# d3sm0/gym_pomdp

Measured on AMD Instinct MI355X. Metric: env steps/sec (whole node), RockSample(7,8) batch=2^20, 1/2/4/8 MI355X, higher is better.
Workload: dtype int32

## Files before the change

### gym_pomdp_amd/csrc/envs/rock.hip.h

```cpp
#pragma once
#include "../envs_common.hip.h"

namespace pomdp {

template <int W, bool STOCH = false>
struct RockEnv {
    using Params = pomdp_rock_params;
    using Reward = int32_t;
    using S = typename std::conditional<W == 1, uint32_t, uint64_t>::type;
    static constexpr int WORDS = W;
    static constexpr const char *NAME = STOCH ? (W == 1 ? "StochasticRockEnv<1>" : "StochasticRockEnv<2>") : (W == 1 ? "RockEnv<1>" : "RockEnv<2>");
    static constexpr bool POOLED_LPT2 = !STOCH;
    static constexpr bool QUAD_STEP = true;
    static constexpr bool HAS_ROCKS = true;
    static constexpr bool POOLED_ANY_LPT = !STOCH;
    static constexpr bool STOCHASTIC = STOCH;
    static constexpr bool QUAD_TAB = true;
    struct Shared {
        uint2 thr[32];
        int8_t grid[256];
        uint8_t rxy[16];
        uint16_t rpos[16];
        uint32_t dir_y[16];
        uint32_t dir_x[16];
// ... 44 lines not shown
        sh.row[tid] = same;
    }

    static __device__ __forceinline__ void load(State &st, const uint32_t *state, int64_t n, uint32_t i)
    {
        st.s = ld_stream(state + i);
        if (W == 2) st.s |= (S)((uint64_t)ld_stream(state + n + i) << 32);
    }
    static __device__ __forceinline__ void store(const State &st, uint32_t *state, int64_t n, uint32_t i, bool)
    {
        st_stream(state + i, (uint32_t)st.s);
        if (W == 2) st_stream(state + n + i, (uint32_t)((uint64_t)st.s >> 32));
    }

    static __device__ __forceinline__ uint32_t elem(const uint4 &w, uint32_t e) { return e == 0 ? w.x : e == 1 ? w.y : e == 2 ? w.z : w.w; }

    template <class LowWord>
    static __device__ __forceinline__ bool k53_le(uint32_t H, uint32_t th, uint32_t tl, LowWord lo)
    {
        const uint32_t kh = H >> 5;
        bool r = kh < th;
        if (kh == th) r = (lo() >> 6) <= tl;
        return r;
    }
    static __device__ __forceinline__ uint32_t rock_code_hi(uint32_t H)
    {
        const uint32_t kh = H >> 5;
        return kh > HALF_HI ? 2u : (kh < HALF_HI ? 0u : 3u);
    }
    static __device__ __forceinline__ uint32_t rock_code_lo(uint32_t L) { return (L >> 6) ? 2u : 1u; }
    template <bool AUTO = false>
    static __device__ __forceinline__ uint4 reset_block(const RngKey &key, uint32_t lane, uint32_t j2)
    {
        const uint32_t c3 = AUTO ? (((uint32_t)POMDP_STREAM_STEP << 24) | (SENSOR_BLOCK + j2)) : (((uint32_t)POMDP_STREAM_RESET << 24) | j2);
        return philox4x32_10(lane >> 2, key.t_lo, key.t_hi, c3, key.k0, key.k1);
    }
    template <bool AUTO>
    static __device__ __forceinline__ uint32_t reset_codes(const RngKey &key, uint32_t lane, int K)
    {
        return reset_codes<AUTO>(elem(reset_block<AUTO>(key, lane, 0u), lane & 3u), key, lane, K);
    }
    template <bool AUTO>
    static __device__ __forceinline__ uint32_t reset_codes(uint32_t w, const RngKey &key, uint32_t lane, int K)
    {
        uint32_t codes = w & 0xAAAAAAAAu;
        if (__popc(w) <= 6) reset_ties<AUTO>(w, key, lane, K, codes, 0);
        return codes & (K >= 16 ? 0xFFFFFFFFu : ((1u << (2 * K)) - 1u));
    }
    template <bool AUTO>
    static __device__ __forceinline__ void reset_ties(uint32_t w, const RngKey &key, uint32_t lane, int K, uint32_t &word, int base)
    {
        bool have_lo = false;
        uint32_t l = 0;
        for (int j = 0; j < K; ++j) {
            const uint32_t rot = (uint32_t)(2 * j + 2) & 31u;
            if (rock_code_hi(__builtin_rotateright32(w, rot)) != 3u) continue;
            if (!have_lo) {
                uint32_t lane_ = lane;
                asm volatile("" : "+v"(lane_));
                l = elem(reset_block<AUTO>(rare_key(key), lane_, 1u), lane & 3u);
                have_lo = true;
            }
            const uint32_t c = rock_code_lo(__builtin_rotateright32(l, rot));
            word = (word & ~(3u << (base + 2 * j))) | (c << (base + 2 * j));
        }
    }
    static __device__ __forceinline__ uint4 quad_block(const RngKey &key, uint32_t lane, uint32_t j2)
    {
        return philox4x32_10(lane >> 2, key.t_lo, key.t_hi, ((uint32_t)POMDP_STREAM_STEP << 24) | j2, key.k0, key.k1);
    }

    static __device__ __forceinline__ void reset_codes4(const uint32_t (&R)[4], const RngKey &key, uint32_t first, int K,
                                                        uint32_t (&codes)[4])
    {
        const uint32_t exist = K >= 16 ? 0xFFFFFFFFu : ((1u << (2 * K)) - 1u);
#pragma unroll
        for (int e = 0; e < 4; ++e) codes[e] = R[e] & 0xAAAAAAAAu & exist;
        if (min(min(__popc(R[0]), __popc(R[1])), min(__popc(R[2]), __popc(R[3]))) <= 6) {
#pragma unroll
            for (int e = 0; e < 4; ++e) codes[e] = reset_codes<true>(R[e], key, first + (uint32_t)e, K);
        }
    }
    static constexpr int RESET_NUMERIC_K = 8;
    static __device__ __forceinline__ uint32_t reset_tie_bound(int K) { return 1u << (2 * min(K, RESET_NUMERIC_K) + 5); }
    template <int N, bool ROT, bool NUMERIC>
    static __device__ __forceinline__ void fresh_states(const uint32_t (&R)[N], const RngKey &key, uint32_t first, int K,
                                                        uint32_t start, uint32_t bound, uint32_t (&fresh)[N])
    {
        const uint32_t exist = K >= 16 ? 0xFFFFFFFFu : ((1u << (2 * K)) - 1u);
        auto word = [&](uint32_t codes) { return ROT ? (codes | start) : (start | (codes << 8)); };
#pragma unroll
        for (int e = 0; e < N; ++e) fresh[e] = word(R[e] & (0xAAAAAAAAu & exist));
        bool look;
        if constexpr (NUMERIC) {
            uint32_t least = R[0];
#pragma unroll
            for (int e = 1; e < N; ++e) least = min(least, R[e]);
            look = least < bound;
        } else {
            int fewest = __popc(R[0]);
#pragma unroll
            for (int e = 1; e < N; ++e) fewest = min(fewest, (int)__popc(R[e]));
            look = fewest <= 6;
        }
        if (look) {
#pragma unroll
            for (int e = 0; e < N; ++e)
                if (__popc(R[e]) <= 6) reset_ties<true>(R[e], key, first + (uint32_t)e, K, fresh[e], ROT ? 0 : 8);
        }
    }
    static __device__ __forceinline__ int reset(const Shared &, const Params &p, State &st, const RngKey &key,
                                                uint32_t lane)
    {
        const uint64_t s = (uint32_t)p.start_x | ((uint32_t)p.start_y << 4);
        st.s = (S)(s | ((uint64_t)reset_codes<false>(key, lane, p.num_rocks) << 8));
        return 0;
    }
    static __device__ __forceinline__ int reset_ob(const Params &, const State &) { return 0; }

    static __device__ __forceinline__ void reset_where(const Shared &, const Params &p, State &st, bool fresh,
                                                       const RngKey &key, uint32_t lane)
    {
        if (!__any(fresh)) return;
        const uint32_t codes = reset_codes<true>(key, lane, p.num_rocks);
        if (fresh) st.s = (S)((uint64_t)((uint32_t)p.start_x | ((uint32_t)p.start_y << 4)) | ((uint64_t)codes << 8));
    }
    static __device__ __forceinline__ void reset_where_chain(const Shared &sh, const Params &p, State &st, bool fresh,
                                                             const RngKey &key, uint32_t lane, const RngKey &akey,
                                                             uint32_t n_actions, int &next_action)
    {
        reset_where_chain_default<RockEnv>(sh, p, st, fresh, key, lane, akey, n_actions, next_action);
    }
    static __device__ __forceinline__ S fresh_state(const Params &p, uint32_t w, const RngKey &key, uint32_t lane)
    {
        return (S)((uint64_t)((uint32_t)p.start_x | ((uint32_t)p.start_y << 4)) | ((uint64_t)reset_codes<true>(w, key, lane, p.num_rocks) << 8));
    }

    static __device__ __forceinline__ int legal_count(const Shared &sh, const Params &p, const State &st, uint32_t &pre,
                                                      int &n_pre, uint32_t &alive)
    {
        const S s = st.s;
        const int x = (int)(s & 15u), y = (int)((s >> 4) & 15u), K = p.num_rocks;
        pre = 1u; n_pre = 1;
        if (y + 1 < p.size) { pre |= 0u << (3 * n_pre); ++n_pre; }
        if (y - 1 >= 0) { pre |= 2u << (3 * n_pre); ++n_pre; }
        if (x - 1 >= 0) { pre |= 3u << (3 * n_pre); ++n_pre; }
        const int id = sh.grid[x * 16 + y];
        if (id >= 0 && id < K && ((uint32_t)(s >> (8 + 2 * (id & 15))) & 3u) != 1u) { pre |= 4u << (3 * n_pre); ++n_pre; }
        const uint64_t r = (uint64_t)s >> 8;
        const uint64_t even = 0x5555555555555555ull;
        const uint64_t spread = ~(r & ~(r >> 1)) & even & ((1ull << (2 * K)) - 1ull);
        alive = (uint32_t)spread;
        return n_pre + __popc(alive);
    }
    struct Legal { uint32_t pre, alive; int n_pre, count; };
    static __device__ __forceinline__ Legal legal_set(const Shared &sh, const Params &p, const State &st)
    {
        Legal L;
        L.count = legal_count(sh, p, st, L.pre, L.n_pre, L.alive);
        return L;
    }
    static __device__ __forceinline__ int legal_pick(const Shared &sh, const Legal &L, int idx)
    {
        if (idx < L.n_pre) return (int)((L.pre >> (3 * idx)) & 7u);
        const int j = nth_set_bit<2>(L.alive, idx - L.n_pre) >> 1;
        const uint32_t rxy = sh.rxy[j & 15];
        return 5 + sh.grid[(rxy & 15u) * 16 + (rxy >> 4)];
    }
    static __device__ __forceinline__ int legal_nth(const Shared &sh, const Params &p, const State &st, int idx)
    {
        return legal_pick(sh, legal_set(sh, p, st), idx);
    }
    static __device__ __forceinline__ int legal_count(const Shared &sh, const Params &p, const State &st)
    {
        uint32_t pre, alive; int n_pre;
        return legal_count(sh, p, st, pre, n_pre, alive);
    }

    static __device__ __forceinline__ bool check_ok(int measured, int count, double pv)
    {
        return measured < 5 && abs(count) < 2 && 0 < pv && pv < 1;
    }
    static __device__ __forceinline__ void belief_update(const Shared &sh, const Params &p, const State &st, int a, int ob,
                                                         const pomdp_rock_belief &b, int64_t n, uint32_t i, uint32_t &ck)
    {
        const S s = st.s;
        const int x = (int)(s & 15u), y = (int)((s >> 4) & 15u), r = (a - 5) & 15;
        const uint32_t rxy = sh.rxy[r];
        const double eff = p.eff[abs(x - (int)(rxy & 15u)) + abs(y - (int)(rxy >> 4))];
        const int64_t k = (int64_t)r * n + i;
        double lkv = b.lkv[k], lkw = b.lkw[k];
// ... 47 lines not shown
        uint32_t m = (alive & ck) << 5;
        if (y + 1 < p.size && north) m |= 1u << 0;
        if (east) m |= 1u << 1;
        if (y - 1 >= 0 && south) m |= 1u << 2;
        if (x - 1 >= 0 && west) m |= 1u << 3;
        return m;
    }

    static __device__ __forceinline__ int select_target(const Shared &sh, const Params &p, const State &st,
                                                        const pomdp_rock_belief &b, int64_t n, uint32_t i)
    {
        const S s = st.s;
        const int x = (int)(s & 15u), y = (int)((s >> 4) & 15u), K = p.num_rocks;
        int best = 4 * p.size * p.size, best_rock = -1;
        for (int j = 0; j < K; ++j) {
            if (((uint32_t)(s >> (8 + 2 * j)) & 3u) == 1u || b.count[(int64_t)j * n + i] < 0) continue;
            const uint32_t rxy = sh.rxy[j];
            const int dx = x - (int)(rxy & 15u), dy = y - (int)(rxy >> 4), d2 = dx * dx + dy * dy;
            if (d2 < best) { best = d2; best_rock = j; }
        }
        return best_rock;
    }

    static __device__ __forceinline__ double compute_prob(const Shared &sh, const Params &p, const State &st, int a, int ob)
    {
        if (a <= 4) return ob == 0 ? 1.0 : 0.0;
        const S s = st.s;
        const int x = (int)(s & 15u), y = (int)((s >> 4) & 15u), r = (a - 5) & 15;
        const uint32_t rxy = sh.rxy[r];
        const double eff = p.eff[abs(x - (int)(rxy & 15u)) + abs(y - (int)(rxy >> 4))];
        const uint32_t code = (uint32_t)(s >> (8 + 2 * r)) & 3u;
        if ((ob == 2 && code == 2u) || (ob == 1 && code == 0u)) return eff;
        return 1 - eff;
    }

    template <class RT>
    static __device__ __forceinline__ void step_pre(const Shared &sh, const Params &p, State &st, int a, RT &rew,
                                                    int &done, Aux &aux)
    {
        const S s = st.s;
        const uint32_t x = (uint32_t)s & 15u, y = ((uint32_t)s >> 4) & 15u;
        const uint32_t size = (uint32_t)p.size, K = (uint32_t)p.num_rocks;
        const int r = (a - 5) & 15;
        const uint32_t rp = sh.rpos[r];
        const uint32_t d = __builtin_amdgcn_sad_u8(x | (y << 8), rp, 0u);
        aux.th = sh.thr[d].x;
        aux.r = (uint8_t)r;
        aux.good = ((uint32_t)(s >> (8 + 2 * r)) & 3u) == 2u;
        aux.want = a > 4;
        const int penalty = STOCH ? 0 : -100;
        const int id = sh.grid[x * 16 + y];
        const int sh_ = 8 + 2 * (id & 15);
        const uint32_t code = (uint32_t)(s >> sh_) & 3u;
        const bool sample_ok = ((uint32_t)id < K) & (code != 1u);
        const uint32_t a2 = (uint32_t)a << 1;
        const uint32_t nx = x + (uint32_t)__builtin_amdgcn_sbfe(0xC4, a2, 2u), ny = y + (uint32_t)__builtin_amdgcn_sbfe(0x31, a2, 2u);
        const bool inside = max(nx, ny) < size;
        const bool is_move = a < 4, is_sample = a == 4, east = a == 1;
        const bool moved = is_move & inside, left = is_move & !inside, sampled = is_sample & sample_ok,
                   missed = is_sample & !sample_ok;
        const uint32_t d_move = ((uint32_t)s & 0xFFu) ^ (nx | (ny << 4));
        const S d_sample = (S)(code ^ 1u) << sh_;
        st.s = s ^ (moved ? (S)d_move : (sampled ? d_sample : (S)0));
        const bool good_rock = code == 2u;
        int rw = ((left & east) | (sampled & good_rock)) ? 10 : 0;
        rw = (sampled & !good_rock) ? -10 : rw;
        rw = ((left & !east) | missed) ? penalty : rw;
        rew = rw;
        if (STOCH) done = left & east;
        else done = left | missed;
    }
    static __device__ __forceinline__ uint32_t thr_lo_of(const Shared &sh, const State &st, int r)
    {
        const uint32_t x = (uint32_t)st.s & 15u, y = ((uint32_t)st.s >> 4) & 15u;
        return sh.thr[__builtin_amdgcn_sad_u8(x | (y << 8), sh.rpos[r & 15], 0u)].y;
    }
    static constexpr int TAB_ACTIONS = W == 1 ? 17 : 21;

    static constexpr uint32_t REC_LUT_LO = 0x0A0A9CF6u, REC_LUT_HI = 0x00000000u;
    using TabEntry = typename std::conditional<W == 1, uint2, uint32_t>::type;
    struct RecTab { TabEntry e[TAB_ACTIONS][256]; };
    static constexpr uint32_t REC_ROCK = 1u << 31;
    static constexpr uint32_t TIE_SPAN = 32u;
    static __device__ __forceinline__ uint32_t rec_thr_word(uint32_t T) { return T >= (1u << 27) ? 0xFFFFFFFFu : T << 5; }
    static __device__ __forceinline__ uint32_t rec_f(uint32_t off, int c, uint32_t ob_mask, uint32_t oc)
    {
        const uint32_t rbyte = (((uint64_t)REC_LUT_HI << 32 | REC_LUT_LO) >> (8u * oc)) & 0xFFu;
        return off | (((uint32_t)c & 3u) << 5) | (ob_mask << 8) | (rbyte << 16) | ((oc & 1u) << 24);
    }
    static constexpr uint32_t ROT_POS = 24u;
    template <bool ROT = false>
    static __device__ __forceinline__ void build_rec_tab(RecTab &tab, const Shared &sh, const Params &p, int pos)
    {
        static_assert(!ROT || W == 1, "the rotated layout is the one-state-word loops'");
        constexpr uint32_t POS0 = ROT ? ROT_POS : 0u, ROCK0 = ROT ? 0u : 8u;
        const uint32_t x = (uint32_t)pos & 15u, y = (uint32_t)pos >> 4, size = (uint32_t)p.size, K = (uint32_t)p.num_rocks;
        const int id = sh.grid[x * 16 + y];
        const uint32_t NOTHING = 6u << 28, PENALTY = (STOCH ? 6u : 1u) << 28, EXIT_EAST = 3u << 28;
        const uint32_t NO_TIE = 1u << 27;
        for (int a = 0; a < 5 + (int)K && a < TAB_ACTIONS; ++a) {
            uint32_t e, f;
            if (a < 4) {
                const uint32_t nx = x + (uint32_t)((a == 1) - (a == 3)), ny = y + (uint32_t)((a == 0) - (a == 2));
                const bool inside = max(nx, ny) < size;
                e = inside ? (((uint32_t)pos ^ (nx | (ny << 4))) | NOTHING) : (a == 1 ? EXIT_EAST : PENALTY);
                e |= NO_TIE;
                f = rec_f(POS0 + ((a & 1) ? 0u : 4u), inside ? (a < 2 ? 1 : -1) : 0, 0u, e >> 28 & 7u);
            } else if (a == 4) {
                const bool rock = (uint32_t)id < K;
                e = (rock ? ((8u + 2u * (uint32_t)id) | 0x80000000u) : 0u) | PENALTY | NO_TIE;
                f = rec_f(rock ? ROCK0 + 2u * (uint32_t)id : 0u, 0, 0u, e >> 28 & 7u);
            } else {
                e = sh.thr[__builtin_amdgcn_sad_u8(x | (y << 8), sh.rpos[a - 5], 0u) & 31u].x | NOTHING;
                f = rec_f(ROCK0 + 2u * (uint32_t)(a - 5), 0, 3u, 6u);
            }
            if constexpr (W == 1) tab.e[a][pos] = make_uint2(a > 4 ? rec_thr_word(e & ~NOTHING) : 0xFFFFFFFFu, f | (a == 4 ? e & REC_ROCK : 0u));
            else tab.e[a][pos] = e;
        }
    }
    template <bool ROT = false>
    static __device__ __forceinline__ uint2 rec_lookup(const RecTab &tab, uint32_t s, uint32_t a)
    {
        if constexpr (ROT) {
            const uint32_t off = __builtin_amdgcn_alignbit(a, s, ROT_POS - 3u) & ~7u;
            return *reinterpret_cast<const uint2 *>(reinterpret_cast<const char *>(&tab.e[0][0]) + off);
        } else return tab.e[a][s & 0xFFu];
    }
    template <bool ROT = false, class LowWord>
    static __device__ __forceinline__ bool rec_sensor_exact(const Shared &sh, uint32_t s, uint32_t f, uint32_t H, LowWord lo)
    {
        const uint32_t pos = ROT ? s >> ROT_POS : s, r = (((f & 31u) - (ROT ? 0u : 8u)) >> 1) & 15u;
        const uint2 t = sh.thr[__builtin_amdgcn_sad_u8((pos & 15u) | ((pos & 0xF0u) << 4), sh.rpos[r], 0u) & 31u];
        const uint32_t kh = H >> 5;
        uint32_t kl = lo() >> 6;
        asm volatile("" : "+v"(kl));
        return kh == t.x ? kl <= t.y : kh < t.x;
    }
    static __device__ __forceinline__ void rec_finish(const uint2 ef, uint32_t &s, uint32_t a, bool correct, uint32_t fresh, uint32_t &rec)
    {
        const uint32_t f = ef.y;
        const uint32_t q = __builtin_amdgcn_ubfe(s, f, 2u);
        const bool ok = ((int32_t)f < 0) & (q != 1u);
        const uint32_t keep = ((q == 2u) == correct) ? 0x7FFFFE00u : 0x7FFFFD00u;
        const uint32_t rfb = (f & keep) | a;
        const uint32_t rok = 0x00F60004u - q * 0x00760000u;
        rec = ok ? rok : rfb;
        const int c = ok ? 1 - (int)q : __builtin_amdgcn_sbfe((int)f, 5u, 2u);
        const uint32_t moved = s + ((uint32_t)c << (f & 31u));
        s = rec >= (1u << 24) ? fresh : moved;
    }
    template <class LowWord>
    static __device__ __forceinline__ void step_rec(const Shared &sh, const RecTab &tab, S &s, uint32_t a, uint32_t H, S fresh,
                                                    uint32_t &rec, LowWord lo)
    {
        const uint32_t s_lo = (uint32_t)s, s_hi = W == 2 ? (uint32_t)((uint64_t)s >> 32) : 0u;
        if constexpr (W == 1) {
            const uint2 ef = rec_lookup(tab, s_lo, a);
            bool correct = H < ef.x;
            if (H - ef.x < TIE_SPAN) correct = rec_sensor_exact(sh, s_lo, ef.y, H, lo);
            uint32_t sn = s_lo;
            rec_finish(ef, sn, a, correct, (uint32_t)fresh, rec);
            s = (S)sn;
        } else {
            const uint32_t e = tab.e[a][s_lo & 0xFFu];
            const bool up_s = (e & 32u) != 0u;
            const uint32_t code = __builtin_amdgcn_ubfe(up_s ? s_hi : s_lo, e, 2u);
            const bool ok = ((int32_t)e < 0) & (code != 1u);
            const uint32_t collect = (code ^ 1u) << (e & 31u);
            const uint32_t move = (a < 4u ? e : 0u) & 0xFFu;
            const uint32_t d_lo = (ok & !up_s) ? collect : move, d_hi = (ok & up_s) ? collect : 0u;
            const uint32_t oc = ok ? code : __builtin_amdgcn_ubfe(e, 28u, 3u);
            const uint32_t rbyte = __builtin_amdgcn_perm(REC_LUT_HI, REC_LUT_LO, (oc << 16) | 0x0C000C0Cu);
            const uint32_t done = oc & 1u;
            const uint32_t gi = 2u * a - 1u;
            const bool good = __builtin_amdgcn_ubfe((gi & 32u) ? s_hi : s_lo, gi, 1u) != 0u;
            const uint32_t kh = __builtin_amdgcn_alignbit(12u, H, 5u);
            bool correct = kh < e;
            if (a > 4u && kh == e) correct = (lo() >> 6) <= thr_lo_of(sh, State{s}, (int)a - 5);
            const uint32_t ob = a > 4u ? ((good == correct) ? 2u << 8 : 1u << 8) : 0u;
            rec = rbyte | (done << 24) | ob | a;
            s = done ? fresh : (S)(((uint64_t)(s_hi ^ d_hi) << 32) | (s_lo ^ d_lo));
        }
    }

    template <class LowWord>
    static __device__ __forceinline__ int sensor_ob(const Shared &sh, const State &st, const Aux &aux, uint32_t H, LowWord lo)
    {
        const uint32_t kh = H >> 5;
        bool correct = kh < aux.th;
        if (kh == aux.th) correct = (lo() >> 6) <= thr_lo_of(sh, st, aux.r);
        return aux.want ? ((aux.good == correct) ? 2 : 1) : 0;
    }

    static constexpr bool QUAD_SENSOR = !STOCH;
    template <class RT>
    static __device__ __forceinline__ void step_with_H(const Shared &sh, const Params &p, State &st, int a, const RngKey &key,
                                                       uint32_t lane, uint32_t H, int &ob, RT &rew, int &done)
    {
        Aux aux;
        step_pre(sh, p, st, a, rew, done, aux);
        ob = sensor_ob(sh, st, aux, H, [&]() { return elem(quad_block(key, lane, 1u), lane & 3u); });
    }

    template <class RT>
    static __device__ __forceinline__ void step(const Shared &sh, const Params &p, State &st, int a,
                                                const RngKey &key, uint32_t lane, int &ob, RT &rew, int &done)
    {
        const uint32_t e = lane & 3u;
        if (STOCH) {
            const uint4 g = quad_block(key, lane, 0u);
            const bool act = k53_le(elem(g, e), (uint32_t)(p.act_thr >> 26), (uint32_t)p.act_thr & LO_MASK,
                                    [&]() { return elem(quad_block(key, lane, 1u), e); }) != (p.act_gt != 0);
            State nx = st;
            Aux aux; RT r2; int d2;
            step_pre(sh, p, nx, a, r2, d2, aux);
            const uint4 h = quad_block(key, lane, 2u);
            const int o2 = sensor_ob(sh, nx, aux, elem(h, e), [&]() { return elem(quad_block(key, lane, 3u), e); });
            if (act) { st = nx; rew = r2; done = d2; ob = o2; }
            else { rew = 0; done = 0; ob = 0; }
            return;
        }
        Aux aux;
        step_pre(sh, p, st, a, rew, done, aux);
        const uint4 h = quad_block(key, lane, 0u);
        ob = sensor_ob(sh, st, aux, elem(h, e), [&]() { return elem(quad_block(key, lane, 1u), e); });
    }
};

}
```

### gym_pomdp_amd/csrc/fused_impl.hip.h

```cpp
#pragma once
#include "kernels_common.hip.h"

namespace pomdp {

template <class L, class Pol, int LPT = 4, bool SROW = false>
struct FusedCtx {
    uint32_t l0, glane0;
    uint64_t t0;
    typename lanes_out<L, LPT, SROW>::type out;
    typename lanes_policy<Pol, LPT>::type pol;
    uint32_t n_bad;
    __device__ __forceinline__ FusedCtx(int32_t *action, int32_t *ob, void *reward, uint8_t *done, int64_t rec, uint32_t lane0,
                                        const RngKey &key0, const RngKey &akey0, uint32_t n_act, int k_steps, const TapeRef &tape)
        : l0(blockIdx.x * (uint32_t)(LPT * BLOCK) + (uint32_t)LPT * threadIdx.x), glane0(lane0 + l0),
          t0(((uint64_t)key0.t_hi << 32) | key0.t_lo), out(action, ob, reward, done, rec, l0),
          pol(tape, l0, glane0, key0, akey0, n_act, k_steps), n_bad(0) {}
    __device__ __forceinline__ void first(int gen_first, int (&a_cur)[LPT])
    {
        if constexpr (LPT == 4) {
            const u32x4 a4 = out.first(pol, gen_first);
#pragma unroll
            for (int j = 0; j < 4; ++j) a_cur[j] = (int)a4[j];
        } else {
            uint32_t a2[LPT];
// ... 182 lines not shown
        if constexpr (quad_policy) {
            if constexpr (!TAPE && !POLICY_WITH_STEP) { if (sj == 0) policy_quarter(s); }
            if constexpr (REC) {
            } else if constexpr (Env::QUAD_SENSOR) {
                const uint32_t rword = pick4(rq);
                st[0].s = fresh[0] ? Env::fresh_state(p, rword, key, glane[0]) : st[0].s;
            } else if constexpr (quad_word_env<Env>::value) {
                Env::fresh_w(sh, p, st[0], fresh[0], key, glane[0], pick4(sq));
            } else {
                Fin::resets_only(sh, p, st, fresh, key, glane);
            }
            const uint32_t word = pick4(aq);
            if constexpr (!TAPE) a_next[0] = (int)__umulhi(word, (uint32_t)n_act);
        } else {
            Fin::run(sh, p, st, fresh, key, glane, akey, (uint32_t)n_act, a_next, aux, o);
        }
#pragma unroll
        for (int j = 0; j < LPT; ++j) {
            if (!live[j]) { o[j] = 0; st[j] = before[j]; }
            if (in_range[j]) out.put_next_action(rel[j], a_next[j]);
            ever_fresh[j] |= fresh[j];
            if (in_range[j]) {
                uint32_t rcode = 0;
                if constexpr (L::CODES && !REC) rcode = Env::reward_code(r[j]);
                if constexpr (REC && L::CODES) out.put_record(j, rel[j], recv[j]);
                else out.put(j, rel[j], a_cur[j], o[j], r[j], rcode, d[j]);
                if (!valid[j] && !was_done[j] && err) atomicAdd(err, 1u);
            }
            if constexpr (TAPE4) a_next[j] = (int)tq[(std::decay_t<decltype(sj_)>::value + 1) & 3];
            else if constexpr (TAPE) a_next[j] = (int)col.nxt;
            a_cur[j] = a_next[j];
            was_done[j] = auto_reset ? false : (d[j] != 0);
        }
        out.next_row();
        if constexpr (Fin::LOOP_BARRIER && !quad_policy) __syncthreads();
    };
    if constexpr (UNROLL4 && UNROLL4_TAIL) {
        #pragma unroll 1
        for (int seg = 0, s = 0; seg < 4; ++seg) {
            const int seg_end = prio.template segment<4>(seg);
            #pragma unroll 1
            for (; s + 4 <= seg_end; s += 4) {
                step_body(s, std::integral_constant<int, 0>{});
                step_body(s + 1, std::integral_constant<int, 1>{});
                step_body(s + 2, std::integral_constant<int, 2>{});
                step_body(s + 3, std::integral_constant<int, 3>{});
            }
            #pragma unroll 1
            for (; s < seg_end; ++s) step_body(s, s & 3);
        }
    } else if constexpr (UNROLL4) {
        #pragma unroll 1
        for (int seg = 0, s = 0; seg < 4; ++seg)
        for (const int seg_end = prio.template segment<4>(seg); s < seg_end; s += 4) {
            step_body(s, std::integral_constant<int, 0>{});
            if (s + 1 < seg_end) {
                step_body(s + 1, std::integral_constant<int, 1>{});
                if (s + 2 < seg_end) {
                    step_body(s + 2, std::integral_constant<int, 2>{});
                    if (s + 3 < seg_end) step_body(s + 3, std::integral_constant<int, 3>{});
                }
            }
        }
    } else {
        #pragma unroll 1
        for (int seg = 0, s = 0; seg < 4; ++seg)
        for (const int seg_end = prio.segment(seg); s < seg_end; ++s) step_body(s, s & 3);
    }
#pragma unroll
    for (int j = 0; j < LPT; ++j)
        if (in_range[j]) { Env::store(st[j], state_w, n, rel[j], ever_fresh[j]); out.finish(j, rel[j], k_steps); }
}

template <class Env, class L, class Pol, int LPT, bool NUMERIC>
__device__ __forceinline__ void steps_quad_body(uint32_t *__restrict__ state, int32_t *__restrict__ action,
                                                int32_t *__restrict__ ob, int32_t *__restrict__ reward,
                                                uint8_t *__restrict__ done, int64_t n, RngKey key0, uint32_t lane0,
                                                RngKey akey0, int k_steps, int64_t rec, int gen_first,
                                                const typename Env::Params &p, TapeRef tape)
{
    static_assert(LPT == 4 || LPT == 2, "a quad or half a quad per thread");
    constexpr int W = Env::WORDS;
    constexpr bool ROT = W == 1;
    using S = typename Env::S;
    __shared__ typename Env::Shared sh;
    __shared__ typename Env::RecTab tab;
    const uint32_t n_act = (uint32_t)Env::n_actions(p);
    constexpr bool AHEAD2 = Pol::TAPE && LPT == 4;
    using PolT = typename std::conditional<AHEAD2, TapeQuadAhead, Pol>::type;
    FusedCtx<L, PolT, LPT, true> cx(action, ob, reward, done, rec, lane0, key0, akey0, n_act, k_steps, tape);
    const uint32_t l0 = cx.l0, glane0 = cx.glane0;
    const uint32_t e0 = LPT == 4 ? 0u : (glane0 & 2u);
    typename Env::State st[LPT];
    int a_cur[LPT];
    uint32_t sp0 = 0, sp1 = 0, gp0 = 0, gp1 = 0;
    {
        uint32_t s_lo[LPT], s_hi[LPT];
        if constexpr (LPT == 4) {
            const u32x4 lo = ld_stream4(state + l0);
            u32x4 hi = {0, 0, 0, 0};
            if (W == 2) hi = ld_stream4(state + n + l0);
#pragma unroll
            for (int j = 0; j < 4; ++j) { s_lo[j] = lo[j]; s_hi[j] = hi[j]; }
        } else {
            const u32x2 lo = ld_stream2(state + l0);
            u32x2 hi = {0, 0};
            if (W == 2) hi = ld_stream2(state + n + l0);
#pragma unroll
            for (int j = 0; j < 2; ++j) { s_lo[j] = lo[j]; s_hi[j] = hi[j]; }
        }
        cx.first(gen_first, a_cur);
#pragma unroll
        for (int j = 0; j < LPT; ++j) {
            if constexpr (ROT) st[j].s = __builtin_amdgcn_alignbit(s_lo[j], s_lo[j], 8u);
            else st[j].s = (S)((uint64_t)s_lo[j] | ((uint64_t)s_hi[j] << 32));
        }
    }
    Env::stage(sh, p, (int)threadIdx.x);
    __syncthreads();
    Env::template build_rec_tab<ROT>(tab, sh, p, (int)threadIdx.x);
    __syncthreads();
    const int K = p.num_rocks;
    const uint32_t start = (uint32_t)p.start_x | ((uint32_t)p.start_y << 4);
    uint32_t start_rot = start << (ROT ? Env::ROT_POS : 0u);
    if constexpr (ROT) asm volatile("" : "+v"(start_rot));
    const LoopPrio prio(k_steps);
    constexpr uint32_t SENSOR_BLOCK = Env::SENSOR_BLOCK;
    const PhiloxFixed sensor_fx = philox_fixed(glane0 >> 2, ((uint32_t)POMDP_STREAM_STEP << 24) | SENSOR_BLOCK, key0.k1);
    const PhiloxFixed gate_fx = philox_fixed(glane0 >> 2, (uint32_t)POMDP_STREAM_STEP << 24, key0.k1);
    uint32_t tie_bound = 0;
    if constexpr (ROT && NUMERIC) { tie_bound = Env::reset_tie_bound(K); asm volatile("" : "+s"(tie_bound)); }
    auto step_body = [&](const int s, const auto par_) __attribute__((always_inline)) {
        constexpr int PAR = decltype(par_)::value;
        const RngKey key = cx.key(key0, s);
        uint32_t H[LPT], G[LPT];
        if constexpr (LPT == 4) {
            const uint4 sw = philox4x32_10_fixed(sensor_fx, key.t_lo, key.t_hi, key.k0, key.k1);
            H[0] = sw.x; H[1] = sw.y; H[2] = sw.z; H[3] = sw.w;
        } else {
            pair_shared(s, e0 != 0u, [&](int sb) { return Env::quad_block(cx.key(key0, sb), glane0, SENSOR_BLOCK); }, H, sp0, sp1);
        }
        uint32_t a_next[LPT];
        if constexpr (AHEAD2) cx.pol.template begin_par<PAR>(s, a_next);
        else cx.pol.begin(s, a_next);
        bool acts[LPT];
#pragma unroll
        for (int j = 0; j < LPT; ++j) acts[j] = true;
        if constexpr (Env::STOCHASTIC) {
            if constexpr (LPT == 4) {
                const uint4 gw = philox4x32_10_fixed(gate_fx, key.t_lo, key.t_hi, key.k0, key.k1);
                G[0] = gw.x; G[1] = gw.y; G[2] = gw.z; G[3] = gw.w;
            } else {
                pair_shared(s, e0 != 0u, [&](int sb) { return Env::quad_block(cx.key(key0, sb), glane0, 0u); }, G, gp0, gp1);
            }
#pragma unroll
            for (int j = 0; j < LPT; ++j)
                acts[j] = Env::k53_le(G[j], (uint32_t)(p.act_thr >> 26), (uint32_t)p.act_thr & Env::LO_MASK,
                                      [&]() { return Env::elem(Env::quad_block(key, glane0, 1u), e0 + (uint32_t)j); }) != (p.act_gt != 0);
        }
        uint32_t rec[LPT], a_taken[LPT];
#pragma unroll
        for (int j = 0; j < LPT; ++j) a_taken[j] = (uint32_t)a_cur[j];
        bool valid[LPT];
#pragma unroll
        for (int j = 0; j < LPT; ++j) valid[j] = !Pol::TAPE || a_taken[j] < n_act;
        auto low_word = [&](int j) __attribute__((always_inline)) {
            return Env::elem(Env::quad_block(rare_key(key), glane0 + (uint32_t)j, SENSOR_BLOCK + 1u), e0 + (uint32_t)j);
        };
        if constexpr (ROT) {
            uint32_t fresh[LPT], sn[LPT];
            uint2 ef[LPT];
            Env::template fresh_states<LPT, true, NUMERIC>(H, key, glane0, K, start_rot, tie_bound, fresh);
#pragma unroll
            for (int j = 0; j < LPT; ++j) ef[j] = Env::template rec_lookup<true>(tab, st[j].s, valid[j] ? a_taken[j] : 0u);
            {
                uint64_t w[LPT];
#pragma unroll
                for (int j = 0; j < LPT; ++j) w[j] = (uint64_t)ef[j].x | ((uint64_t)ef[j].y << 32);
                if constexpr (LPT == 4) asm volatile("" : "+v"(w[0]), "+v"(w[1]), "+v"(w[2]), "+v"(w[3]));
                else asm volatile("" : "+v"(w[0]), "+v"(w[1]));
#pragma unroll
                for (int j = 0; j < LPT; ++j) ef[j] = make_uint2((uint32_t)w[j], (uint32_t)(w[j] >> 32));
            }
            uint32_t near[LPT];
            bool correct[LPT];
#pragma unroll
            for (int j = 0; j < LPT; ++j) correct[j] = __builtin_sub_overflow(H[j], ef[j].x, &near[j]);
            uint32_t nearest = near[0];
#pragma unroll
            for (int j = 1; j < LPT; ++j) nearest = min(nearest, near[j]);
            if (nearest < Env::TIE_SPAN) {
#pragma unroll
                for (int j = 0; j < LPT; ++j)
                    if (near[j] < Env::TIE_SPAN)
                        correct[j] = Env::template rec_sensor_exact<true>(sh, st[j].s, ef[j].y, H[j], [&]() { return low_word(j); });
            }
#pragma unroll
            for (int j = 0; j < LPT; ++j) {
                sn[j] = st[j].s;
                Env::rec_finish(ef[j], sn[j], valid[j] ? a_taken[j] : 0u, correct[j], fresh[j], rec[j]);
            }
#pragma unroll
            for (int j = 0; j < LPT; ++j) {
                if constexpr (Env::STOCHASTIC) {
                    sn[j] = acts[j] ? sn[j] : st[j].s;
                    rec[j] = acts[j] ? rec[j] : a_taken[j];
                }
                if constexpr (Pol::TAPE) {
                    sn[j] = valid[j] ? sn[j] : st[j].s;
                    rec[j] = valid[j] ? rec[j] : a_taken[j];
                    cx.n_bad += (uint32_t)!valid[j];
                }
                st[j].s = sn[j];
            }
        } else {
            uint32_t codes[LPT];
            if constexpr (LPT == 4) Env::reset_codes4(H, key, glane0, K, codes);
            else {
#pragma unroll
                for (int j = 0; j < LPT; ++j) codes[j] = Env::template reset_codes<true>(H[j], key, glane0 + (uint32_t)j, K);
            }
#pragma unroll
            for (int j = 0; j < LPT; ++j) {
                S sj = st[j].s;
                Env::step_rec(sh, tab, sj, valid[j] ? a_taken[j] : 0u, H[j], (S)((uint64_t)start | ((uint64_t)codes[j] << 8)), rec[j],
                              [&]() { return low_word(j); });
                if constexpr (Env::STOCHASTIC) {
                    sj = acts[j] ? sj : st[j].s;
                    rec[j] = acts[j] ? rec[j] : a_taken[j];
                }
                if constexpr (Pol::TAPE) {
                    sj = valid[j] ? sj : st[j].s;
                    rec[j] = valid[j] ? rec[j] : a_taken[j];
                    cx.n_bad += (uint32_t)!valid[j];
                }
                st[j].s = sj;
            }
        }
        cx.out.put_records(rec, a_next);
        if constexpr (AHEAD2) {
            cx.pol.template end_par<PAR>(s, a_next);
#pragma unroll
            for (int j = 0; j < LPT; ++j) a_cur[j] = (int)a_next[j];
        } else cx.advance(s, a_next, a_cur);
    };
    if constexpr (AHEAD2) {
        wait_loads();
        _Pragma("unroll 1") for (int seg = 0, s = 0; seg < 4; ++seg)
            for (const int seg_end = prio.template segment<2>(seg); s < seg_end; s += 2) {
                step_body(s, std::integral_constant<int, 0>{});
                if (s + 1 < seg_end) step_body(s + 1, std::integral_constant<int, 1>{});
            }
    } else {
        POMDP_FUSED_STEP_LOOP(prio, s) step_body(s, std::integral_constant<int, 0>{});
    }
    cx.finish(k_steps);
    uint32_t w_lo[LPT];
#pragma unroll
    for (int j = 0; j < LPT; ++j) w_lo[j] = ROT ? __builtin_amdgcn_alignbit((uint32_t)st[j].s, (uint32_t)st[j].s, 24u) : (uint32_t)st[j].s;
    if constexpr (LPT == 4) {
        st_stream4(state + l0, w_lo[0], w_lo[1], w_lo[2], w_lo[3]);
        if (W == 2)
            st_stream4(state + n + l0, (uint32_t)((uint64_t)st[0].s >> 32), (uint32_t)((uint64_t)st[1].s >> 32),
                       (uint32_t)((uint64_t)st[2].s >> 32), (uint32_t)((uint64_t)st[3].s >> 32));
    } else {
        st_stream2(state + l0, w_lo[0], w_lo[1]);
        if (W == 2) st_stream2(state + n + l0, (uint32_t)((uint64_t)st[0].s >> 32), (uint32_t)((uint64_t)st[1].s >> 32));
    }
}
template <class Env, class L = Columns, class Pol = SyntheticQuad, int LPT = 4>
__global__ __launch_bounds__(BLOCK) void steps_quad_kernel(uint32_t *__restrict__ state, int32_t *__restrict__ action,
                                                           int32_t *__restrict__ ob, int32_t *__restrict__ reward,
                                                           uint8_t *__restrict__ done, int64_t n, RngKey key0, uint32_t lane0,
                                                           RngKey akey0, int k_steps, int64_t rec, int gen_first,
                                                           const typename Env::Params p, TapeRef tape)
{
    steps_quad_body<Env, L, Pol, LPT, Env::WORDS == 1>(state, action, ob, reward, done, n, key0, lane0, akey0, k_steps, rec, gen_first, p, tape);
}
template <class Env, class L = Columns, class Pol = SyntheticQuad, int LPT = 4>
__global__ __launch_bounds__(BLOCK) void steps_quad_popc_kernel(uint32_t *__restrict__ state, int32_t *__restrict__ action,
                                                                int32_t *__restrict__ ob, int32_t *__restrict__ reward,
                                                                uint8_t *__restrict__ done, int64_t n, RngKey key0, uint32_t lane0,
                                                                RngKey akey0, int k_steps, int64_t rec, int gen_first,
                                                                const typename Env::Params p, TapeRef tape)
{
    static_assert(Env::WORDS == 1, "two state words take reset_codes4");
    steps_quad_body<Env, L, Pol, LPT, false>(state, action, ob, reward, done, n, key0, lane0, akey0, k_steps, rec, gen_first, p, tape);
}

template <bool TAB, class L = Columns, class Pol = SyntheticQuad, int LPT = 4>
__global__ __launch_bounds__(BLOCK) void tag_steps_quad_kernel(uint32_t *__restrict__ state, int32_t *__restrict__ action,
                                                               int32_t *__restrict__ ob, float *__restrict__ reward,
                                                               uint8_t *__restrict__ done, int64_t n, RngKey key0,
                                                               uint32_t lane0, RngKey akey0, int k_steps, int64_t rec,
                                                               int gen_first, const TagEnv::Params p, TapeRef tape)
{
    using Env = TagEnv;
    static_assert(LPT == 4 || LPT == 2, "a quad or half a quad per thread");
    __shared__ Env::Shared sh;
    __shared__ typename std::conditional<TAB, Env::StepTab, NoTab>::type tab;
    const uint32_t n_act = (uint32_t)Env::n_actions(p);
    FusedCtx<L, Pol, LPT> cx(action, ob, reward, done, rec, lane0, key0, akey0, n_act, k_steps, tape);
    const uint32_t l0 = cx.l0, glane0 = cx.glane0;
    const uint32_t e0 = LPT == 4 ? 0u : (glane0 & 2u);
    Env::State st[LPT];
    int a_cur[LPT];
    uint32_t sp0 = 0, sp1 = 0;
    {
        if constexpr (LPT == 4) {
            const u32x4 s4 = ld_stream4(state + l0);
            cx.first(gen_first, a_cur);
#pragma unroll
            for (int j = 0; j < 4; ++j) st[j].w = s4[j];
        } else {
            const u32x2 s2 = ld_stream2(state + l0);
            cx.first(gen_first, a_cur);
#pragma unroll
            for (int j = 0; j < 2; ++j) st[j].w = s2[j];
        }
    }
    Env::stage(sh, p, (int)threadIdx.x);
    __syncthreads();
    if constexpr (TAB) {
        Env::build_tab(tab, sh, p, (int)threadIdx.x);
        __syncthreads();
    }
    const LoopPrio prio(k_steps);
    POMDP_FUSED_STEP_LOOP(prio, s) {
        const RngKey key = cx.key(key0, s);
        uint32_t a_next[LPT];
        cx.pol.begin(s, a_next);
        int o[LPT], d[LPT];
        float r[LPT];
        uint32_t a_taken[LPT], W[LPT];
#pragma unroll
        for (int j = 0; j < LPT; ++j) a_taken[j] = (uint32_t)a_cur[j];
        if constexpr (LPT == 4) {
            const uint4 qw = Env::quad_block(key, glane0, 0u);
            W[0] = qw.x; W[1] = qw.y; W[2] = qw.z; W[3] = qw.w;
        } else {
            pair_shared(s, e0 != 0u, [&](int sb) { return Env::quad_block(cx.key(key0, sb), glane0, 0u); }, W, sp0, sp1);
        }
// ... 724 lines not shown
```

### gym_pomdp_amd/envs/rock.py

```python
import ctypes as C

import torch

from .. import _native, tables
from .base import BatchedEnv, staggered


class _BeliefTracker(object):
    FIELDS = (("count", torch.int32), ("measured", torch.int32), ("lkv", torch.float64), ("lkw", torch.float64),
              ("prob_valuable", torch.float64))

    def __init__(self, env):
        self.env = env
        k, n = env.num_rocks, env.batch_size
        cols = staggered([((k, n), dt) for _, dt in self.FIELDS] + [((n,), torch.int32)], env.device)
        self.tensors = {f: c for (f, _), c in zip(self.FIELDS, cols)}
        self.check_ok = cols[-1]
        self.ptrs = _native.RockBelief(*([self.tensors[f].data_ptr() for f, _ in self.FIELDS] + [self.check_ok.data_ptr()]))
        self.ref = C.byref(self.ptrs)
        self.on_reset()

    def on_reset(self, where=None):
        env = self.env
        with torch.cuda.device(env.device):
            rc = env._lib.pomdp_rock_belief_reset(env._params_ref, self.ref, None if where is None else where.data_ptr(),
                                                  env.batch_size, env._stream())
        _native.check(rc, "pomdp_rock_belief_reset")

    def on_step(self, action, ob, done, flags):
        env = self.env
        with torch.cuda.device(env.device):
            rc = env._lib.pomdp_rock_belief_update(env._params_ref, env._state.data_ptr(), action.data_ptr(),
                                                   ob.data_ptr(), done.data_ptr(), self.ref, env.batch_size, flags,
                                                   env._stream())
        if rc:
            _native.check(rc, "pomdp_rock_belief_update")


def make_params(board_size=7, num_rocks=8, stochastic=False, p_move=.8):
    assert board_size in tables.ROCK_CONFIG and num_rocks in tables.ROCK_CONFIG[board_size][0], \
        "unsupported RockSample(%r, %r)" % (board_size, num_rocks)
    _, init_pos, rock_pos = tables.ROCK_CONFIG[board_size]
    if num_rocks > len(rock_pos):
        raise IndexError("RockSample(%d,%d): only %d rock positions are configured"
                         % (board_size, num_rocks, len(rock_pos)))
    p = _native.RockParams()
    p.size, p.num_rocks = board_size, num_rocks
    p.start_x, p.start_y = init_pos
    for i in range(256):
        p.grid[i] = -1
    for idx, (x, y) in enumerate(rock_pos):
        p.grid[x * 16 + y] = idx
        p.rock_x[idx], p.rock_y[idx] = x, y
    for d in range(32):
        p.thr[d] = tables.ROCK_THR[min(d, len(tables.ROCK_THR) - 1)]
        p.eff[d] = tables.ROCK_EFF[min(d, len(tables.ROCK_EFF) - 1)]
    if stochastic:
        p.stochastic = 1
        if p_move == .8:
            p.act_thr = tables.TAG_MOVE_THR
        else:
            if not 0. < p_move < 1.:
                raise ValueError("StochasticRock: p_move must lie in (0, 1), got %r" % (p_move,))
            thr, sense = tables.bernoulli_threshold(p_move)
            p.act_thr, p.act_gt = thr, int(sense == "gt")
    words = 1 if num_rocks <= 12 else 2
    return p, words, 5 + num_rocks, 3


class RockEnv(BatchedEnv):
    env_name = "rock"
    reward_dtype = torch.int32

    def __init__(self, board_size=7, num_rocks=8, use_heuristic=False, track_belief=None, **batch_kwargs):
        self.board_size = board_size
        self.num_rocks = num_rocks
        self.p_move = getattr(self, "p_move", None)
        self._use_heuristic = use_heuristic
        self._discount = .95
        self._reward_range = 20
        self._penalization = -100
        self._setup(**batch_kwargs)
        if use_heuristic if track_belief is None else track_belief:
            with torch.cuda.device(self.device):
                self._tracker = _BeliefTracker(self)

    @property
    def belief(self):
        return None if self._tracker is None else self._tracker.tensors

    def _belief_ref(self):
        if self._tracker is None:
            raise RuntimeError("RockEnv: side statistics are not tracked (construct with use_heuristic=True or "
                               "track_belief=True)")
        return self._tracker.ref

    def set_belief(self, belief):
        for f, _ in _BeliefTracker.FIELDS:
            self._tracker.tensors[f].copy_(torch.as_tensor(belief[f], device=self.device).reshape(self.num_rocks, -1))
        with torch.cuda.device(self.device):
            rc = self._lib.pomdp_rock_belief_refresh(self._params_ref, self._tracker.ref, self.batch_size, self._stream())
            _native.check(rc, "pomdp_rock_belief_refresh")

    def _generate_preferred(self, history):
        if not self._use_heuristic:
            return self._generate_legal()
        return super()._generate_preferred(history)

    def select_target(self, state=None):
        st = self._state if state is None else self._checked_state(state, self.batch_size, "select_target")
        out = torch.empty(self.batch_size, dtype=torch.int32, device=self.device)
        with torch.cuda.device(self.device):
            rc = self._lib.pomdp_rock_select_target(self._params_ref, st.data_ptr(), self._belief_ref(), out.data_ptr(),
                                                    self.batch_size, self._stream())
            _native.check(rc, "pomdp_rock_select_target")
        return out

    def _select_target(self, rock_state=None, x_size=None):
        t = self.select_target(rock_state)
        return int(t.item()) if self.batch_size == 1 else t

    def _build_params(self):
        return make_params(self.board_size, self.num_rocks)

    def _validate_state(self, st, what):
        w = st[0].to(torch.int64)
        if bool((((w & 15) >= self.board_size) | (((w >> 4) & 15) >= self.board_size)).any()):
            raise ValueError("%s: RockSample state with the agent off the %d x %d board" % (what, self.board_size, self.board_size))

    def decode_state(self):
        s = self._state.to(torch.int64) & 0xFFFFFFFF
        v = s[0] if self.state_words == 1 else (s[0] | (s[1] << 32))
        cols = [v & 15, (v >> 4) & 15] + [((v >> (8 + 2 * j)) & 3) - 1 for j in range(self.num_rocks)]
        return torch.stack(cols, dim=1)

    def _decode_state(self, state, as_array=True):
        s = torch.as_tensor(state, device=self.device).to(torch.int64).reshape(-1, 1 + self.num_rocks)
        v = (s[:, 0] % self.board_size) | ((s[:, 0] // self.board_size) << 4)
        for j in range(self.num_rocks):
# ... 20 lines not shown
```

Baseline: 967.1 billion.

## Use bitfield-insert state layout for rotated numeric RockSample step path

```diff
diff --git a/gym_pomdp_amd/csrc/envs/rock.hip.h b/gym_pomdp_amd/csrc/envs/rock.hip.h
--- a/gym_pomdp_amd/csrc/envs/rock.hip.h
+++ b/gym_pomdp_amd/csrc/envs/rock.hip.h
@@ -150,15 +150,21 @@
         }
     }
     static constexpr int RESET_NUMERIC_K = 8;
+    static constexpr uint32_t INS_ROCK0 = 5u;
     static __device__ __forceinline__ uint32_t reset_tie_bound(int K) { return 1u << (2 * min(K, RESET_NUMERIC_K) + 5); }
-    template <int N, bool ROT, bool NUMERIC>
+    template <int N, bool ROT, bool NUMERIC, bool INS = false>
     static __device__ __forceinline__ void fresh_states(const uint32_t (&R)[N], const RngKey &key, uint32_t first, int K,
                                                         uint32_t start, uint32_t bound, uint32_t (&fresh)[N])
     {
+        static_assert(!INS || (ROT && NUMERIC), "the insert layout is the rotated one of the boards with at most RESET_NUMERIC_K rocks");
         const uint32_t exist = K >= 16 ? 0xFFFFFFFFu : ((1u << (2 * K)) - 1u);
+        constexpr int ROCK0 = INS ? (int)INS_ROCK0 : ROT ? 0 : 8;
         auto word = [&](uint32_t codes) { return ROT ? (codes | start) : (start | (codes << 8)); };
 #pragma unroll
-        for (int e = 0; e < N; ++e) fresh[e] = word(R[e] & (0xAAAAAAAAu & exist));
+        for (int e = 0; e < N; ++e) {
+            if constexpr (INS) fresh[e] = ((R[e] << INS_ROCK0) & ((0xAAAAAAAAu & exist) << INS_ROCK0)) | start;
+            else fresh[e] = word(R[e] & (0xAAAAAAAAu & exist));
+        }
         bool look;
         if constexpr (NUMERIC) {
             uint32_t least = R[0];
@@ -174,7 +180,7 @@
         if (look) {
 #pragma unroll
             for (int e = 0; e < N; ++e)
-                if (__popc(R[e]) <= 6) reset_ties<true>(R[e], key, first + (uint32_t)e, K, fresh[e], ROT ? 0 : 8);
+                if (__popc(R[e]) <= 6) reset_ties<true>(R[e], key, first + (uint32_t)e, K, fresh[e], ROCK0);
         }
     }
     static __device__ __forceinline__ int reset(const Shared &, const Params &p, State &st, const RngKey &key,
@@ -388,60 +394,65 @@
     struct RecTab { TabEntry e[TAB_ACTIONS][256]; };
     static constexpr uint32_t REC_ROCK = 1u << 31;
     static constexpr uint32_t TIE_SPAN = 32u;
-    static __device__ __forceinline__ uint32_t rec_thr_word(uint32_t T) { return T >= (1u << 27) ? 0xFFFFFFFFu : T << 5; }
+    template <bool INS = false>
+    static __device__ __forceinline__ uint32_t rec_thr_word(uint32_t T) { return T >= (1u << 27) ? (INS ? 0xFFFFFFE0u : 0xFFFFFFFFu) : T << 5; }
     static __device__ __forceinline__ uint32_t rec_f(uint32_t off, int c, uint32_t ob_mask, uint32_t oc)
     {
         const uint32_t rbyte = (((uint64_t)REC_LUT_HI << 32 | REC_LUT_LO) >> (8u * oc)) & 0xFFu;
         return off | (((uint32_t)c & 3u) << 5) | (ob_mask << 8) | (rbyte << 16) | ((oc & 1u) << 24);
     }
     static constexpr uint32_t ROT_POS = 24u;
-    template <bool ROT = false>
+    template <bool ROT = false, bool INS = false>
     static __device__ __forceinline__ void build_rec_tab(RecTab &tab, const Shared &sh, const Params &p, int pos)
     {
         static_assert(!ROT || W == 1, "the rotated layout is the one-state-word loops'");
-        constexpr uint32_t POS0 = ROT ? ROT_POS : 0u, ROCK0 = ROT ? 0u : 8u;
+        static_assert(!INS || ROT, "the insert layout is a rotated one");
+        constexpr uint32_t POS0 = ROT ? ROT_POS : 0u, ROCK0 = INS ? INS_ROCK0 : ROT ? 0u : 8u;
         const uint32_t x = (uint32_t)pos & 15u, y = (uint32_t)pos >> 4, size = (uint32_t)p.size, K = (uint32_t)p.num_rocks;
         const int id = sh.grid[x * 16 + y];
         const uint32_t NOTHING = 6u << 28, PENALTY = (STOCH ? 6u : 1u) << 28, EXIT_EAST = 3u << 28;
         const uint32_t NO_TIE = 1u << 27;
         for (int a = 0; a < 5 + (int)K && a < TAB_ACTIONS; ++a) {
-            uint32_t e, f;
+            uint32_t e, f, ins = 0u;
             if (a < 4) {
                 const uint32_t nx = x + (uint32_t)((a == 1) - (a == 3)), ny = y + (uint32_t)((a == 0) - (a == 2));
                 const bool inside = max(nx, ny) < size;
                 e = inside ? (((uint32_t)pos ^ (nx | (ny << 4))) | NOTHING) : (a == 1 ? EXIT_EAST : PENALTY);
                 e |= NO_TIE;
-                f = rec_f(POS0 + ((a & 1) ? 0u : 4u), inside ? (a < 2 ? 1 : -1) : 0, 0u, e >> 28 & 7u);
+                f = rec_f(POS0 + ((a & 1) ? 0u : 4u), inside && !INS ? (a < 2 ? 1 : -1) : 0, 0u, e >> 28 & 7u);
+                if (inside) ins = (((a & 1) ? nx : ny) << (f & 31u)) | 4u;
             } else if (a == 4) {
                 const bool rock = (uint32_t)id < K;
                 e = (rock ? ((8u + 2u * (uint32_t)id) | 0x80000000u) : 0u) | PENALTY | NO_TIE;
                 f = rec_f(rock ? ROCK0 + 2u * (uint32_t)id : 0u, 0, 0u, e >> 28 & 7u);
+                if (rock) ins = (1u << (f & 31u)) | 2u;
             } else {
                 e = sh.thr[__builtin_amdgcn_sad_u8(x | (y << 8), sh.rpos[a - 5], 0u) & 31u].x | NOTHING;
                 f = rec_f(ROCK0 + 2u * (uint32_t)(a - 5), 0, 3u, 6u);
             }
-            if constexpr (W == 1) tab.e[a][pos] = make_uint2(a > 4 ? rec_thr_word(e & ~NOTHING) : 0xFFFFFFFFu, f | (a == 4 ? e & REC_ROCK : 0u));
+            if constexpr (W == 1) tab.e[a][pos] = make_uint2(a > 4 ? rec_thr_word<INS>(e & ~NOTHING) : INS ? ins : 0xFFFFFFFFu, f | (a == 4 ? e & REC_ROCK : 0u));
             else tab.e[a][pos] = e;
         }
     }
-    template <bool ROT = false>
+    template <bool ROT = false, bool INS = false>
     static __device__ __forceinline__ uint2 rec_lookup(const RecTab &tab, uint32_t s, uint32_t a)
     {
         if constexpr (ROT) {
-            const uint32_t off = __builtin_amdgcn_alignbit(a, s, ROT_POS - 3u) & ~7u;
+            const uint32_t off = __builtin_amdgcn_alignbit(a, s, ROT_POS - 3u) & (INS ? ~0u : ~7u);
             return *reinterpret_cast<const uint2 *>(reinterpret_cast<const char *>(&tab.e[0][0]) + off);
         } else return tab.e[a][s & 0xFFu];
     }
-    template <bool ROT = false, class LowWord>
+    template <bool ROT = false, bool INS = false, class LowWord>
     static __device__ __forceinline__ bool rec_sensor_exact(const Shared &sh, uint32_t s, uint32_t f, uint32_t H, LowWord lo)
     {
-        const uint32_t pos = ROT ? s >> ROT_POS : s, r = (((f & 31u) - (ROT ? 0u : 8u)) >> 1) & 15u;
+        const uint32_t pos = ROT ? s >> ROT_POS : s, r = (((f & 31u) - (INS ? INS_ROCK0 : ROT ? 0u : 8u)) >> 1) & 15u;
         const uint2 t = sh.thr[__builtin_amdgcn_sad_u8((pos & 15u) | ((pos & 0xF0u) << 4), sh.rpos[r], 0u) & 31u];
         const uint32_t kh = H >> 5;
         uint32_t kl = lo() >> 6;
         asm volatile("" : "+v"(kl));
         return kh == t.x ? kl <= t.y : kh < t.x;
     }
+    template <bool INS = false>
     static __device__ __forceinline__ void rec_finish(const uint2 ef, uint32_t &s, uint32_t a, bool correct, uint32_t fresh, uint32_t &rec)
     {
         const uint32_t f = ef.y;
@@ -451,8 +462,16 @@
         const uint32_t rfb = (f & keep) | a;
         const uint32_t rok = 0x00F60004u - q * 0x00760000u;
         rec = ok ? rok : rfb;
-        const int c = ok ? 1 - (int)q : __builtin_amdgcn_sbfe((int)f, 5u, 2u);
-        const uint32_t moved = s + ((uint32_t)c << (f & 31u));
+        uint32_t moved;
+        if constexpr (INS) {
+            uint32_t m;
+            asm("v_bfm_b32 %0, %1, %2" : "=v"(m) : "v"(ef.x), "v"(f));
+            asm("v_bfi_b32 %0, %1, %2, %3" : "=v"(moved) : "v"(m), "v"(ef.x), "v"(s));
+            asm("" : "+v"(rec));
+        } else {
+            const int c = ok ? 1 - (int)q : __builtin_amdgcn_sbfe((int)f, 5u, 2u);
+            moved = s + ((uint32_t)c << (f & 31u));
+        }
         s = rec >= (1u << 24) ? fresh : moved;
     }
     template <class LowWord>
diff --git a/gym_pomdp_amd/csrc/fused_impl.hip.h b/gym_pomdp_amd/csrc/fused_impl.hip.h
--- a/gym_pomdp_amd/csrc/fused_impl.hip.h
+++ b/gym_pomdp_amd/csrc/fused_impl.hip.h
@@ -288,6 +288,7 @@
     static_assert(LPT == 4 || LPT == 2, "a quad or half a quad per thread");
     constexpr int W = Env::WORDS;
     constexpr bool ROT = W == 1;
+    constexpr bool INS = ROT && NUMERIC;
     using S = typename Env::S;
     __shared__ typename Env::Shared sh;
     __shared__ typename Env::RecTab tab;
@@ -318,13 +319,14 @@
         cx.first(gen_first, a_cur);
 #pragma unroll
         for (int j = 0; j < LPT; ++j) {
-            if constexpr (ROT) st[j].s = __builtin_amdgcn_alignbit(s_lo[j], s_lo[j], 8u);
+            if constexpr (INS) st[j].s = (s_lo[j] << Env::ROT_POS) | ((s_lo[j] >> (8u - Env::INS_ROCK0)) & (0xFFFFu << Env::INS_ROCK0));
+            else if constexpr (ROT) st[j].s = __builtin_amdgcn_alignbit(s_lo[j], s_lo[j], 8u);
             else st[j].s = (S)((uint64_t)s_lo[j] | ((uint64_t)s_hi[j] << 32));
         }
     }
     Env::stage(sh, p, (int)threadIdx.x);
     __syncthreads();
-    Env::template build_rec_tab<ROT>(tab, sh, p, (int)threadIdx.x);
+    Env::template build_rec_tab<ROT, INS>(tab, sh, p, (int)threadIdx.x);
     __syncthreads();
     const int K = p.num_rocks;
     const uint32_t start = (uint32_t)p.start_x | ((uint32_t)p.start_y << 4);
@@ -376,9 +378,9 @@
         if constexpr (ROT) {
             uint32_t fresh[LPT], sn[LPT];
             uint2 ef[LPT];
-            Env::template fresh_states<LPT, true, NUMERIC>(H, key, glane0, K, start_rot, tie_bound, fresh);
-#pragma unroll
-            for (int j = 0; j < LPT; ++j) ef[j] = Env::template rec_lookup<true>(tab, st[j].s, valid[j] ? a_taken[j] : 0u);
+            Env::template fresh_states<LPT, true, NUMERIC, INS>(H, key, glane0, K, start_rot, tie_bound, fresh);
+#pragma unroll
+            for (int j = 0; j < LPT; ++j) ef[j] = Env::template rec_lookup<true, INS>(tab, st[j].s, valid[j] ? a_taken[j] : 0u);
             {
                 uint64_t w[LPT];
 #pragma unroll
@@ -399,12 +401,12 @@
 #pragma unroll
                 for (int j = 0; j < LPT; ++j)
                     if (near[j] < Env::TIE_SPAN)
-                        correct[j] = Env::template rec_sensor_exact<true>(sh, st[j].s, ef[j].y, H[j], [&]() { return low_word(j); });
+                        correct[j] = Env::template rec_sensor_exact<true, INS>(sh, st[j].s, ef[j].y, H[j], [&]() { return low_word(j); });
             }
 #pragma unroll
             for (int j = 0; j < LPT; ++j) {
                 sn[j] = st[j].s;
-                Env::rec_finish(ef[j], sn[j], valid[j] ? a_taken[j] : 0u, correct[j], fresh[j], rec[j]);
+                Env::template rec_finish<INS>(ef[j], sn[j], valid[j] ? a_taken[j] : 0u, correct[j], fresh[j], rec[j]);
             }
 #pragma unroll
             for (int j = 0; j < LPT; ++j) {
@@ -463,7 +465,11 @@
     cx.finish(k_steps);
     uint32_t w_lo[LPT];
 #pragma unroll
-    for (int j = 0; j < LPT; ++j) w_lo[j] = ROT ? __builtin_amdgcn_alignbit((uint32_t)st[j].s, (uint32_t)st[j].s, 24u) : (uint32_t)st[j].s;
+    for (int j = 0; j < LPT; ++j) {
+        const uint32_t sj = (uint32_t)st[j].s;
+        w_lo[j] = INS ? (sj >> Env::ROT_POS) | ((sj & (0xFFFFu << Env::INS_ROCK0)) << (8u - Env::INS_ROCK0))
+                      : ROT ? __builtin_amdgcn_alignbit(sj, sj, 24u) : sj;
+    }
     if constexpr (LPT == 4) {
         st_stream4(state + l0, w_lo[0], w_lo[1], w_lo[2], w_lo[3]);
         if (W == 2)
diff --git a/gym_pomdp_amd/envs/rock.py b/gym_pomdp_amd/envs/rock.py
--- a/gym_pomdp_amd/envs/rock.py
+++ b/gym_pomdp_amd/envs/rock.py
@@ -55,6 +55,7 @@
     for d in range(32):
         p.thr[d] = tables.ROCK_THR[min(d, len(tables.ROCK_THR) - 1)]
         p.eff[d] = tables.ROCK_EFF[min(d, len(tables.ROCK_EFF) - 1)]
+        assert 1 << 52 <= p.thr[d] <= 1 << 53, (d, p.thr[d])
     if stochastic:
         p.stochastic = 1
         if p_move == .8:
```

Result: faster. 992.5 billion, median of 6 (+2.6%).
